# ojcharles/WeightedLD

Hardware: AMD Instinct MI355X
Metric: LD site-pairs/sec at N=2000 seq × L=20000 var sites; 1/2/4/8 GPU; %HBM roofline (higher is better)
Workload: dtype fp6 (e2m3) weights x fp4 (e2m1) codes on block-scaled MFMA, screen (f32 sums, exact on the rounded weights; rigorous f32 r2 bound over every pair); candidate tiles (0 of 49144): f32 sums in lib.rs's order on f32 MFMA, f32 epilogue

## Files before the change

include/weightedld.h:

```cpp
#ifndef WEIGHTEDLD_H
#define WEIGHTEDLD_H

#include <stddef.h>
#include <stdint.h>

#ifdef __cplusplus
extern "C" {
#endif

#define WLD_OK 0
#define WLD_E_ARG (-1)
#define WLD_E_HIP (-2)
#define WLD_E_OOM (-3)
#define WLD_E_NODEV (-4)
#define WLD_E_IO (-5)
#define WLD_E_FORMAT (-6)
#define WLD_E_STATE (-7)

#define WLD_SYM_A 0
#define WLD_SYM_C 1
#define WLD_SYM_G 2
#define WLD_SYM_T 3
#define WLD_SYM_MISSING 4
#define WLD_SYM_UNKNOWN 5
// ... 51 lines not shown
#define WLD_OPT_MFMA_LAYOUT 5
#define WLD_OPT_VALU_PLAIN 6
#define WLD_OPT_STAGING_ROWS 7
#define WLD_OPT_HOST_BATCH_PAIRS 8
#define WLD_OPT_REF_SUMS 11
#define WLD_OPT_FUSED_SCAN 12
#define WLD_OPT_SCREEN_FP6 13
#define WLD_OPT_TEST_GUARD 14
#define WLD_OPT_FP6_PAIRS_MIN_TILES 15
#define WLD_OPT_I8_PAIRS 16
#define WLD_OPT_FP6_A4 17
#define WLD_OPT_TARGET_BATCH_SLOTS 18
#define WLD_OPT_FP6_SHARED 19
#define WLD_OPT_PARTNERS_BATCH_BYTES 20
#define WLD_OPT_FP6_THREE 21
int wld_set_option(wld_ctx *ctx, int option, int64_t value);
int wld_get_option(wld_ctx *ctx, int option, int64_t *value);

int wld_set_window(wld_ctx *ctx, uint64_t max_distance, uint64_t max_sites);
int wld_get_window(wld_ctx *ctx, uint64_t *max_distance, uint64_t *max_sites);
int wld_window_pairs_in_chunks(wld_ctx *ctx, uint32_t begin, uint32_t end, uint64_t *pairs);
int wld_shard_chunks_window(wld_ctx *ctx, int n_shards, int shard, uint32_t *begin, uint32_t *end);
int wld_window_limits_copy(wld_ctx *ctx, uint32_t *hi);

typedef struct {
    uint64_t n;
    uint32_t *site_a;
    uint32_t *site_b;
    float *d;
    float *d_prime;
// ... 61 lines not shown
    int mfma_planes;
    uint64_t tiles;
    uint64_t candidate_tiles;
    double screen_ms;
    int screened;
    int ref_sums;
    uint64_t candidate_blocks;
    uint64_t candidate_pairs;
    int screen_fp6;
    int fp6_sampled;
    uint64_t progress_filled;
    int fp6_a4;
    int fp6_shared;
    int fp6_three;
    uint64_t fp6_rechecked;
} wld_run_stats;
int wld_last_stats(wld_ctx *ctx, wld_run_stats *out);
int wld_fp6_weight_codes(wld_ctx *ctx, uint8_t *codes, int *fits_fp4);

typedef struct {
    uint64_t n_sites;
    uint64_t bin_width;
    uint32_t n_bins;
    uint64_t pairs, none_pairs, nonfinite_pairs, counted_pairs;
    double r2_sum;
    double *score;
    uint32_t *partners;
    uint64_t *bin_pairs;
    double *bin_r2_sum;
    double kernel_ms;
// ... 133 lines not shown
```

weightedld_amd/_lib.py:

```python
import ctypes
import os

PKG_DIR = os.path.dirname(os.path.abspath(__file__))
LIB_PATH = os.environ.get("WLD_LIB_PATH") or os.path.join(PKG_DIR, "libweightedld.so")

WLD_OK = 0
STATUS = {
    -1: "WLD_E_ARG",
    -2: "WLD_E_HIP",
    -3: "WLD_E_OOM",
    -4: "WLD_E_NODEV",
    -5: "WLD_E_IO",
    -6: "WLD_E_FORMAT",
    -7: "WLD_E_STATE",
}
KERNEL_AUTO, KERNEL_VALU, KERNEL_MFMA = 0, 1, 2
OPTIONS = {"prefilter": 1, "screen": 2, "tile_order": 3, "all_planes": 4, "mfma_layout": 5, "valu_plain": 6,
           "staging_rows": 7, "host_batch_pairs": 8, "ref_sums": 11, "fused_scan": 12, "screen_fp6": 13,
           "test_guard": 14, "fp6_pairs_min_tiles": 15, "i8_pairs": 16, "fp6_a4": 17,
           "target_batch_slots": 18, "fp6_shared": 19, "partners_batch_bytes": 20, "fp6_three": 21}


class WldError(RuntimeError):
    def __init__(self, status, where, message):
        self.status = status
        self.name = STATUS.get(status, str(status))
        super().__init__("%s: %s (%s)" % (where, message, self.name))


class Pairs(ctypes.Structure):
    _fields_ = [
        ("n", ctypes.c_uint64),
        ("site_a", ctypes.POINTER(ctypes.c_uint32)),
        ("site_b", ctypes.POINTER(ctypes.c_uint32)),
        ("d", ctypes.POINTER(ctypes.c_float)),
# ... 15 lines not shown
        ("mfma_planes", ctypes.c_int),
        ("tiles", ctypes.c_uint64),
        ("candidate_tiles", ctypes.c_uint64),
        ("screen_ms", ctypes.c_double),
        ("screened", ctypes.c_int),
        ("ref_sums", ctypes.c_int),
        ("candidate_blocks", ctypes.c_uint64),
        ("candidate_pairs", ctypes.c_uint64),
        ("screen_fp6", ctypes.c_int),
        ("fp6_sampled", ctypes.c_int),
        ("progress_filled", ctypes.c_uint64),
        ("fp6_a4", ctypes.c_int),
        ("fp6_shared", ctypes.c_int),
        ("fp6_three", ctypes.c_int),
        ("fp6_rechecked", ctypes.c_uint64),
    ]


class Summary(ctypes.Structure):
    _fields_ = [
        ("n_sites", ctypes.c_uint64),
        ("bin_width", ctypes.c_uint64),
        ("n_bins", ctypes.c_uint32),
        ("pairs", ctypes.c_uint64),
        ("none_pairs", ctypes.c_uint64),
        ("nonfinite_pairs", ctypes.c_uint64),
        ("counted_pairs", ctypes.c_uint64),
        ("r2_sum", ctypes.c_double),
        ("score", ctypes.POINTER(ctypes.c_double)),
        ("partners", ctypes.POINTER(ctypes.c_uint32)),
# ... 283 lines not shown
```

weightedld_amd/csrc/capi.hip:

```cpp
#include <algorithm>
#include <cmath>
#include <chrono>
#include <condition_variable>
#include <cstdlib>
#include <cstring>
#include <deque>
#include <functional>
#include <mutex>
#include <string>
#include <thread>
#include <vector>

#include "common.hpp"
#include "tile_order.hpp"
#include "window_plan.hpp"
#include "summary_plan.hpp"
#include "heatmap_plan.hpp"
#include "annot_plan.hpp"
#include "blocks_plan.hpp"
#include "partners_plan.hpp"
#include "prune_plan.hpp"
#include "targets_plan.hpp"
#include "kernels.hpp"
#include "fp6_scale.hpp"
// ... 75 lines not shown
    unsigned long long *d_hcnt = nullptr;
    int cand_set = 0;
    int kernel_pref = WLD_KERNEL_AUTO;
    bool opt_prefilter = true, opt_tile_rows = false, opt_all_planes = false;
    int opt_screen = 1;
    screen_policy::Learned learned;
    screen_policy::Plan pass;
    DevBuf fp6_probe_buf;
    bool opt_site_major = false, opt_valu_plain = false;
    bool opt_fused_scan = true;
    int opt_test_guard = 0;
    int64_t opt_fp6_pairs_min = 0;
    bool opt_i8_pairs = true;
    int opt_fp6 = 1;
    bool opt_fp6_a4 = true;
    int opt_fp6_three = 1;
    bool opt_fp6_shared = true;
    bool opt_ref_sums = true;
    uint64_t opt_staging_rows = 1ull << 25, opt_host_batch_pairs = 1ull << 31;
    uint64_t opt_target_slots = targets_plan::kDefaultBatchSlots;
    uint64_t opt_partners_bytes = partners_plan::kDefaultBatchBytes;

    bool loaded = false;
    size_t L = 0, N = 0, LP = 0, NP = 0;
    DevBuf raw, wraw, codes, w_pad, wstats, site_ok, site_map, planes, frag;
    DevBuf rcodes, rw;
    DevBuf w6, f6a, f6b, f6marg;
    DevBuf w4;
    Fp6Screen f6{};
    DevBuf i8a, i8b;
// ... 517 lines not shown
double ref_extra_residual(const wld_ctx *c) {
    const double u = 0x1p-24, m = (double)(c->N / 8) + 16.0;
    const double gamma = m * u / (1.0 - m * u);
    double qsum = 0.0;
    for (int p = 0; p < 4; ++p) qsum += std::ldexp((double)c->wst.dsum[p], 8 * p);
    const double r = 9.0 * gamma * (qsum + 0.5 * (double)c->N) + 0.5 * (double)c->N;
    return r * (1.0 + 1e-9) + 1.0;
}

struct PolicyInputs {
    screen_policy::Options opt;
    screen_policy::LoadFacts load;
    screen_policy::PassFacts pass;
};
PolicyInputs policy_inputs(const wld_ctx *c, float thr, bool dense) {
    return {{c->opt_screen, c->opt_fp6, c->opt_ref_sums, c->opt_prefilter, c->opt_i8_pairs, c->opt_fp6_three},
            {c->kernel == WLD_KERNEL_MFMA, c->use_frag, c->wst.nonneg != 0, c->NP, c->plane_mask, c->fp6_ok,
             c->fp6_better},
            {c->f6_n_pairs != 0, c->n_tiles, thr, dense, c->prog_pass, c->pend.count_out != nullptr}};
}

ValuLaunch ref_valu_launch(wld_ctx *c, float thr) {
    return ValuLaunch{ptr<uint8_t>(c->rcodes), ptr<float>(c->rw), ptr<uint8_t>(c->site_ok), ptr<uint32_t>(c->tiles),
                      c->n_tiles, nullptr, (uint32_t)c->L, (uint32_t)c->NPr, chunk_rows_of(c->L), thr, c->safe, false,
                      true, c->ref_cls, (uint32_t)(c->N % 8)};
}

MfmaLaunch mfma_base(wld_ctx *c, float thr) {
    MfmaLaunch m{};
    m.wplanes = ptr<int8_t>(c->planes);
    m.tiles = ptr<uint32_t>(c->tiles);
// ... 33 lines not shown
        launch_pair_valu(ValuLaunch{ptr<uint8_t>(c->codes), ptr<float>(c->w_pad), ptr<uint8_t>(c->site_ok),
                                    ptr<uint32_t>(c->tiles), c->n_tiles, nullptr, (uint32_t)c->L, (uint32_t)c->NP,
                                    chunk_rows_of(c->L), thr, c->safe, c->opt_valu_plain, false, 0, 0},
                         o, dense, c->stream);
    } else {
        MfmaLaunch m = mfma_base(c, thr);
        m.codes = ptr<uint8_t>(c->codes);
        m.frag = c->use_frag ? ptr<uint8_t>(c->frag) : nullptr;
        m.frag_b = c->use_frag ? ptr<uint8_t>(c->frag) + c->LP * c->NP : nullptr;
        m.shift = c->shift;
        m.plane_mask = c->plane_mask;
        m.route = plan.route;
        m.bound_test = plan.bound_test;
        m.fp6_bail = plan.fp6_bail;
        m.fp6_three = plan.fp6_three;
        m.f6_rechecked = reinterpret_cast<unsigned *>(ptr<unsigned long long>(c->counters) + kF6Rechecked);
        m.i8img = &c->i8s;
        for (int t = 0; t < 3; ++t) m.resid[t] = c->wst.resid[t];
        for (int p = 0; p < 4; ++p) m.dsum[p] = c->wst.dsum[p];
        m.cand_list = ptr<uint32_t>(c->cand);
        unsigned long long *set = ptr<unsigned long long>(c->counters) + kCandSet0 + kCandSetWords * c->cand_set;
        m.cand_count = reinterpret_cast<unsigned *>(set);
        m.cand_work = reinterpret_cast<unsigned *>(ptr<unsigned long long>(c->counters) + 2) + 1;
        m.cand_buckets = reinterpret_cast<unsigned *>(set + 1);
        m.test_guard = c->opt_test_guard;
        if (scan && !dense) m.scan = *scan;
        RefRowsLaunch rr{};
        if (c->opt_ref_sums) {
            m.ref_valu = &rv;
            m.r_extra_q = ref_extra_residual(c);
// ... 148 lines not shown
            c->learned.reset();
            break;
        case WLD_OPT_FP6_A4:
            c->opt_fp6_a4 = value != 0;
            c->fp6_ok = c->fp6_better = c->fp6_tried = false;
            break;
        case WLD_OPT_FP6_SHARED:
            c->opt_fp6_shared = value != 0;
            c->fp6_ok = c->fp6_better = c->fp6_tried = false;
            break;
        case WLD_OPT_FP6_THREE:
            if (value < 0 || value > 2) return fail(WLD_E_ARG, "WLD_OPT_FP6_THREE takes 0 to 2");
            c->opt_fp6_three = (int)value;
            c->learned.reset();
            break;
        default: return fail(WLD_E_ARG, "unknown option %d", option);
    }
    return WLD_OK;
}

int wld_fp6_weight_codes(wld_ctx *c, uint8_t *codes, int *fits_fp4) {
    if (!c || !codes || !fits_fp4) return fail(WLD_E_ARG, "null argument");
    if (!c->members.empty()) return fail(WLD_E_ARG, "wld_fp6_weight_codes takes a single-device context");
    if (c->pend.active) return fail(WLD_E_STATE, "wld_fp6_weight_codes during a run");
    if (!c->loaded || !c->fp6_ok) return fail(WLD_E_STATE, "the loaded set has no fp6 operands");
    HIP_TRY(hipSetDevice(c->device));
    HIP_TRY(hipMemcpyAsync(codes, c->w6.p, c->N, hipMemcpyDeviceToHost, c->stream));
    HIP_TRY(hipStreamSynchronize(c->stream));
    *fits_fp4 = fp6_codes_fit_fp4(codes, c->N) ? 1 : 0;
    return WLD_OK;
// ... 83 lines not shown
        case WLD_OPT_MFMA_LAYOUT: *value = c->opt_site_major; break;
        case WLD_OPT_VALU_PLAIN: *value = c->opt_valu_plain; break;
        case WLD_OPT_REF_SUMS: *value = c->opt_ref_sums; break;
        case WLD_OPT_STAGING_ROWS: *value = (int64_t)c->opt_staging_rows; break;
        case WLD_OPT_HOST_BATCH_PAIRS: *value = (int64_t)c->opt_host_batch_pairs; break;
        case WLD_OPT_TARGET_BATCH_SLOTS: *value = (int64_t)c->opt_target_slots; break;
        case WLD_OPT_PARTNERS_BATCH_BYTES: *value = (int64_t)c->opt_partners_bytes; break;
        case WLD_OPT_FUSED_SCAN: *value = c->opt_fused_scan; break;
        case WLD_OPT_TEST_GUARD: *value = c->opt_test_guard; break;
        case WLD_OPT_FP6_PAIRS_MIN_TILES: *value = c->opt_fp6_pairs_min; break;
        case WLD_OPT_SCREEN_FP6: *value = c->opt_fp6; break;
        case WLD_OPT_I8_PAIRS: *value = c->opt_i8_pairs; break;
        case WLD_OPT_FP6_A4: *value = c->opt_fp6_a4; break;
        case WLD_OPT_FP6_SHARED: *value = c->opt_fp6_shared; break;
        case WLD_OPT_FP6_THREE: *value = c->opt_fp6_three; break;
        default: return fail(WLD_E_ARG, "unknown option %d", option);
    }
    return WLD_OK;
}

int wld_load(wld_ctx *c, const uint8_t *sites, size_t n_sites, size_t n_seqs, const uint64_t *site_map,
             const float *weights) {
    if (c && !c->members.empty()) {
        const size_t G = c->members.size();
        std::vector<int> st(G, WLD_OK);
        std::vector<std::string> msg(G);
        std::vector<std::thread> th;
        for (size_t k = 0; k < G; ++k)
            th.emplace_back([&, k] {
                st[k] = wld_load(c->members[k], sites, n_sites, n_seqs, site_map, weights);
// ... 248 lines not shown
        launch_gather(o, ptr<uint32_t>(c->chunk_base), r.lin_begin, lin_count, chunk_rows_of(c->L), (uint32_t)c->L, 0,
                      cn, c->out_a.bytes / 4, c->has_map && !c->prune_run ? ptr<uint32_t>(c->site_map) : nullptr,
                      ptr<uint32_t>(c->out_a), ptr<uint32_t>(c->out_b), ptr<float>(c->out_d), ptr<float>(c->out_dp),
                      ptr<float>(c->out_r2), c->stream);
        HIP_TRY(hipGetLastError());
        HIP_TRY(hipEventRecord(c->ev[5], c->stream));
        c->gather_cap = c->out_a.bytes / 4;
    }
    return WLD_OK;
}

int fp6_sample(wld_ctx *c, float thr, bool operands_fresh) {
    const PolicyInputs in = policy_inputs(c, thr, false);
    if (!screen_policy::wants_sample(in.opt, in.load, in.pass, c->learned)) return WLD_OK;
    const hipStream_t s = !operands_fresh && c->own_stream ? c->own_stream : c->stream;
    WLD_TRY(ensure(c->fp6_probe_buf, 3 * sizeof(unsigned)));
    MfmaLaunch m = mfma_base(c, thr);
    m.fp6_three = c->opt_fp6_three != 0 && m.f6_pairs != nullptr;
    const uint32_t entries = m.f6_pairs ? m.f6_n_pairs : m.n_tiles;
    const uint32_t stride = std::max<uint32_t>(1, std::min<uint32_t>(64, entries / 256));
    launch_fp6_probe(m, ptr<unsigned>(c->fp6_probe_buf), stride, s);
    HIP_TRY(hipGetLastError());
    unsigned h[3] = {0, 0, 0};
    HIP_TRY(hipMemcpyAsync(h, c->fp6_probe_buf.p, sizeof(h), hipMemcpyDeviceToHost, s));
    HIP_TRY(hipStreamSynchronize(s));
    c->fp6_sampled = true;
    screen_policy::learn(c->learned, screen_policy::Sample{thr, h[0], h[1], m.fp6_three, h[2]});
    return WLD_OK;
}

int run_enqueue(wld_ctx *c, float thr, uint32_t lin_begin, uint32_t lin_end, unsigned long long *count_out) {
    const uint32_t n = chunk_rows_of(c->L);
    c->have_rows = false;
    c->pend.active = false;
    const bool fp6_fresh = !c->fp6_tried && c->opt_fp6 != 0;
    if (fp6_fresh) WLD_TRY(fp6_prepare(c));
    WLD_TRY(build_tiles(c, lin_begin, lin_end, true));
    c->fp6_sampled = false;
    WLD_TRY(fp6_sample(c, thr, fp6_fresh));
    const uint64_t pairs = run_pairs(c, lin_begin, lin_end);
    const uint32_t T = (uint32_t)(c->LP / kTile);
    const uint32_t n_chunks = n * (n + 1) / 2;
// ... 145 lines not shown
    c->spec_gather = rows > 0;
    c->gather_cap = 0;
    c->stats.kernel = c->kernel;
    c->stats.pairs = r.pairs;
    c->stats.rows = rows;
    c->times_pending = true;
    c->times_order_end = order_end;
    c->stats.pair_kernel_launches = c->n_tiles ? screen_policy::stat_launches(route) : 0;
    c->stats.tiles = c->tiles_windowed ? c->n_tiles_listed : c->n_tiles;
    c->stats.screened = screen_policy::stat_screened(route);
    c->stats.screen_fp6 = screen_policy::stat_screen_fp6(route) ? 1 : abandoned ? 2 : 0;
    c->stats.fp6_sampled = c->fp6_sampled ? 1 : 0;
    c->stats.fp6_a4 = c->stats.screen_fp6 == 1 && c->f6.a4 ? 1 : 0;
    c->stats.fp6_shared = c->stats.screen_fp6 == 1 && c->f6.shared ? 1 : 0;
    c->stats.fp6_three = c->stats.screen_fp6 == 1 ? screen_policy::stat_fp6_three(c->pass) : 0;
    c->stats.fp6_rechecked = c->stats.fp6_three ? __atomic_load_n(&c->h_cnt[5], __ATOMIC_ACQUIRE) : 0;
    c->stats.candidate_pairs = cand_pairs ? h[0] : 0;
    screen_policy::learn(c->learned, screen_policy::Outcome{route, r.thr, false, h[2], c->n_tiles, h[0], r.pairs});
    c->stats.candidate_tiles = screened ? h[2] : c->n_tiles;
    c->stats.candidate_blocks = screened && !cand_pairs ? h[3] : 16 * (uint64_t)c->n_tiles;
    if (n_rows) *n_rows = rows;
    return WLD_OK;
}

int run_chunks(wld_ctx *c, float thr, uint32_t lin_begin, uint32_t lin_end, uint64_t *n_rows) {
    WLD_TRY(run_enqueue(c, thr, lin_begin, lin_end, nullptr));
    return run_complete(c, n_rows);
}
}

int wld_run(wld_ctx *c, float thr, uint32_t rb, uint32_t re, uint64_t *n_rows) {
// ... 1992 lines not shown
```

weightedld_amd/csrc/kernels.hpp:

```cpp
#pragma once

#include <hip/hip_runtime.h>

#include <cstdint>
#include <vector>

#include "screen_policy.hpp"

namespace wld {

constexpr int kChunk = 256;
constexpr int kTile = 64;
constexpr int kSeqPad = 64;
constexpr int kTilesPerChunk = kChunk / kTile;
constexpr uint32_t kNoTile = 0xFFFFFFFFu;

constexpr uint8_t kCodeIn = 1;
constexpr uint8_t kCodeMaj = 2;

struct OrderArgs {
    uint32_t *st_a, *st_b;
    float *st_d, *st_dp, *st_r2;
    uint64_t st_capacity;
    uint8_t *seg_cnt;
// ... 275 lines not shown
    uint32_t *cand_list;
    unsigned *cand_count;
    unsigned *cand_buckets;
    int test_guard = 0;
    unsigned *cand_work;
    const ValuLaunch *ref_valu;
    double r_extra_q;
    const RefRowsLaunch *ref_rows;
    ScanArgs scan;
    const Fp6Screen *fp6;
    uint32_t fp6_bail;
    const uint32_t *f6_pairs;
    uint32_t f6_n_pairs;
    bool fp6_three = false;
    unsigned *f6_rechecked = nullptr;
    const I8Screen *i8img = nullptr;
};
void launch_fp6_probe(const MfmaLaunch &m, unsigned *probe, uint32_t stride, hipStream_t s);
void launch_pair_mfma(const MfmaLaunch &m, const OrderArgs &o, const DenseArgs *dense, hipStream_t s,
                      hipEvent_t screen_done);

void launch_progress_init(unsigned *chunk_left, uint32_t lin_begin, uint32_t count, uint32_t n_chunk_rows, uint32_t L,
                          unsigned *prog_n, hipStream_t s);
void launch_progress_init_window(unsigned *chunk_left, uint32_t lin_begin, uint32_t count, uint32_t n_chunk_rows,
                                 const uint32_t *tiles, uint32_t n_tiles, unsigned *prog_n, hipStream_t s);
void launch_window_limits(const uint32_t *pos, uint32_t L, uint32_t LP, uint64_t D, uint64_t K, uint32_t *hi,
                          hipStream_t s);
void launch_run_init(unsigned long long *counters, uint32_t *chunk_total, uint32_t n_chunks, hipStream_t s);
void launch_chunk_scan(const ScanArgs &a, hipStream_t s);
void launch_gather(const OrderArgs &o, const uint32_t *chunk_base, uint32_t lin_begin, uint32_t count,
// ... 33 lines not shown
```

weightedld_amd/csrc/pair_common.hpp:

```cpp
#pragma once

#include "kernels.hpp"

namespace wld {

#ifndef WLD_EPI_DIVT
#define WLD_EPI_DIVT 1
#endif
__host__ __device__ __forceinline__ double recip_f64(double t, double r0) {
    double r = r0;
    double e = fma(-t, r, 1.0);
    r = fma(r, e, r);
    e = fma(-t, r, 1.0);
    return fma(r, e, r);
}
__host__ __forceinline__ double recip_seed_host(float t) {
    return fabsf(t) < 0x1p-126f ? (double)(1.0f / (t * 0x1p64f)) * 0x1p64 : (double)(1.0f / t);
}
__host__ __device__ __forceinline__ void ld_epilogue(float total_weight, float PA, float PB, float ld3, float &d_out,
                                                     float &dp_out, float &r2_out) {
    float ld_obs0, ld_obs1, ld_obs2, ld_obs3 = ld3;
    float Pa = total_weight - PA;
    float Pb = total_weight - PB;
    ld_obs2 = PA - ld_obs3;
// ... 146 lines not shown
    return F6tCol{col + mb, col - mb, fmaf(2.0f, mb, -R2), 2.0f * Mb, mb, col};
}
__host__ __device__ __forceinline__ float r2_screen_terms_f6t(float p, float s, float t, const F6tRow &a,
                                                              const F6tCol &b, float thr_c, float E, float &mlo) {
    const float d = s - t;
    const float m1 = a.c1 - d, m2 = (a.rA2 + b.cB2) + d;
    const float m3 = fmaf(2.0f, p, a.rA + b.cB3), m4 = fmaf(-2.0f, p, b.c4);
    mlo = fminf(fminf(m1, m2), fminf(m3, m4));
    const float cap2 = fminf(fmaf(-2.0f, p, a.Ma2), b.Mb2 - d);
    const float q = -((a.ma2 - s) * (b.mb - p));
    const float X0lo = p + (a.row + b.col);
    const float nt = fmaxf(fabsf(fmaf(X0lo, t, q)), fabsf(fmaf(X0lo + cap2, t, q)));
    const float nub = fmaf(2.0f, nt, E);
    return fmaf(nub, nub, -(thr_c * ((m1 * m2) * (m3 * m4))));
}
__host__ __device__ __forceinline__ float r2_screen_violation(float T, float A, float B, float AB, float R,
                                                              float thr_c) {
    float E, mloc, t2;
    screen_consts(T, R, E, mloc);
    const float t1 = r2_screen_terms(T, A, B, AB, R, thr_c, E, mloc, t2);
    return fmaxf(t1, t2);
}
__host__ __device__ __forceinline__ bool r2_screen_skip_f32(float T, float A, float B, float AB, float R, float thr) {
    return r2_screen_violation(T, A, B, AB, R, thr * (1.0f - 0x1p-7f)) <= 0.0f;
}
constexpr uint32_t kScreenF32MaxNP = 32768;

__device__ __forceinline__ void glds16(const void *gsrc, uint32_t lds_dst) {
    uint32_t keep;
    asm volatile(
// ... 101 lines not shown
        *a.cursor = 0;
        unsigned cand = 0, blocks = 0;
        if (a.cand_count) {
            cand = ld32(a.cand_count);
            blocks = ld32(a.cand_count + 1);
        }
        if (a.cursor_seen) *a.cursor_seen = (cand & kAbandonBit) ? ~0ull : cur;
        if (a.cand_reset) a.cand_reset[0] = a.cand_reset[1] = 0;
        if (a.cand_buckets_reset)
            for (int b = 0; b < 16; ++b) a.cand_buckets_reset[b] = 0;
        if (a.host_out) {
            a.host_out[0] = cur;
            a.host_out[1] = run;
            a.host_out[2] = cand;
            a.host_out[3] = blocks;
            if (a.rechecked) a.host_out[5] = ld32(a.rechecked);
            __threadfence_system();
        }
        if (a.rechecked) *a.rechecked = 0;
    }
    __syncthreads();
    unsigned long long base = sw[wv] + v - s;
    if (in_regs) {
#pragma unroll
        for (uint32_t j = 0; j < kScanRegs; ++j)
            if (lo + j < hi) {
                ct[lo + j] = 0;
                a.chunk_base[lo + j] = (uint32_t)base;
                base += vals[j];
            }
        return;
    }
    for (uint32_t i = lo; i < hi; ++i) {
        const uint32_t t = ld32(ct + i);
// ... 56 lines not shown
```

weightedld_amd/csrc/pair_mfma.hip:

```cpp
#include <algorithm>
#include <type_traits>
#include <vector>

#include "fp6_pack.hpp"
#include "pair_common.hpp"


namespace wld {

typedef int v4i __attribute__((ext_vector_type(4)));
typedef int v16i __attribute__((ext_vector_type(16)));

bool mfma_supported() { return true; }

namespace {
constexpr int kGroup = 8;
constexpr int kStageCodes = 4096;
constexpr int kDigStage = 128;
constexpr int kMaxPlanes = 4;
constexpr uint32_t kPlanes012 = 0 | (1 << 2) | (2 << 4);
constexpr int kDigGroup = 1024;
template <int NPL>
struct GroupShape {
    static constexpr int kStages = NPL == 1 ? 4 : kGroup;
// ... 844 lines not shown
    }
    bool doubt = false;
#pragma unroll
    for (int e = 0; e < 4; ++e) {
        const float2 a = sA[16 * ep.wq + 4 * (ep.lane >> 4) + e];
        const F6tRow ra = f6t_row(W6, a.x, a.y, ep.R2);
#pragma unroll
        for (int n = 0; n < 4; ++n) {
            float mlo;
            const float t1 = terms(ra, n, e, mlo);
            if (ep.valid_pair(4 * n + e) && (t1 > 0.0f || !(mlo >= ep.mloc))) doubt = true;
        }
    }
    return doubt;
}
}

template <int kFmt>
__global__ __launch_bounds__(256, 4) void pair_fp6_screen_kernel(const uint8_t *__restrict__ a6,
                                                                  const uint8_t *__restrict__ b6,
                                                                  const float2 *__restrict__ marg, float W6,
                                                                  const uint64_t *__restrict__ ok_bits,
                                                                  const uint32_t *__restrict__ tiles, uint32_t n_tiles,
                                                                  uint32_t NK, uint32_t L, uint32_t n_chunk_rows,
                                                                  float thr, OrderArgs o, ScreenArgs sc, float wv) {
    using F = F6Fmt<kFmt>;
    constexpr int kF6AStage = F::kAStage, kF6ABytes = F::kABytes, kF6Stage = F::kStage;
    __shared__ __attribute__((aligned(16))) uint8_t smem[2 * kF6Stage];
    __shared__ float2 sMarg[2 * kTile];
    __shared__ unsigned long long sMask;
// ... 74 lines not shown
        screen_verdict((uint32_t)sMask, ta, tb, tid, n_chunk_rows, o, sc);
    } else {
        screen_verdict(0u, ta, tb, tid, n_chunk_rows, o, sc);
    }
}

constexpr uint32_t kF6Single = 0x8000u;

#ifdef WLD_EXP_CLOCK
constexpr uint32_t kF6ClockSlots = 8192;
__device__ unsigned long long gF6Clock[2 * kF6ClockSlots];
extern "C" int wld_debug_f6_clock(unsigned long long *out) {
    return (int)hipMemcpyFromSymbol(out, HIP_SYMBOL(gF6Clock), sizeof(gF6Clock));
}
#endif
template <int kFmt, bool kThree = false>
__global__ __launch_bounds__(256, 3) void pair_fp6_screen2w_kernel(
    const uint8_t *__restrict__ a6, const uint8_t *__restrict__ b6, const float2 *__restrict__ marg, float W6,
    const uint64_t *__restrict__ ok_bits,
    const uint32_t *__restrict__ pairs, uint32_t n_pairs, uint32_t NK, uint32_t L, uint32_t n_chunk_rows, float thr,
    OrderArgs o, ScreenArgs sc, float wv) {
    using F = F6Fmt<kFmt>;
    constexpr int kF6AStage = F::kAStage, kF6ABytes = F::kABytes, kF6PStage = F::kPStage;
    __shared__ __attribute__((aligned(16))) uint8_t smem[2 * kF6PStage];
    __shared__ float2 sMarg[3 * kTile];
    __shared__ unsigned long long sMask[2];
    __shared__ uint32_t sBail, sCand[2];
    __shared__ uint32_t sDoubt[2];
    if (!sc.probe && blockIdx.x == 0 && threadIdx.x == 0) *sc.cand_work = 0u;
    const uint32_t tid = threadIdx.x, lane = tid & 63, wave = __builtin_amdgcn_readfirstlane(tid >> 6);
    const uint32_t half = wave >> 1, rp = wave & 1, ltid = tid & 127;
    const uint32_t lds = lds_addr(smem), lane16 = lane * 16;
    const uint32_t ei = sc.probe ? blockIdx.x * sc.probe_stride + blockIdx.x % sc.probe_stride : blockIdx.x;
    const uint32_t entry = ei < n_pairs ? pairs[ei] : kNoTile;
    if (entry == kNoTile) return;
    constexpr int kAPieces = kFmt == kF6A6 ? 3 : kFmt == kF6A4 ? 2 : 1;
    static_assert(kF6AStage == kAPieces * 4096 && kF6BStage == 4096, "five (fp4 A: four, shared: three) pieces per wave and stage");
    struct Src {
        const uint8_t *pA, *pB0, *pB1;
    };
    auto src_of = [&](uint32_t e) {
        const uint32_t ta_ = e >> 16, tb0_ = e & 0x7FFFu;
        Src r;
// ... 21 lines not shown
        const uint32_t tb = tb0 + (idle ? 0u : half);
        if (tid < 3 * kTile) {
            const uint32_t t = tid < kTile ? ta : tb0 + ((tid >= 2 * kTile && !single) ? 1u : 0u);
            sMarg[tid] = marg[t * kTile + (tid & (kTile - 1))];
        }
        if (tid == 0) {
            uint32_t v = 0;
            if (sc.bail) {
                const unsigned cc = __hip_atomic_load(sc.cand_count, __ATOMIC_RELAXED, __HIP_MEMORY_SCOPE_AGENT);
                v = cc > sc.bail ? ((cc & kAbandonBit) ? 2u : 1u) : 0u;
            }
            sBail = v;
        }
        if constexpr (kThree)
            if (tid < 2) sDoubt[tid] = 0u;
        asm volatile("s_waitcnt lgkmcnt(0)" ::: "memory");
        const uint64_t okA = ok_bits[ta], okB = ok_bits[tb];
        v4f acc[2][4][2][2];
        const uint32_t boff = kF6AStage + (idle ? 0u : half) * kF6BStage;
        const uint32_t aoff = 2 * rp * kF6ABytes;
        auto stage = [&](uint32_t kb, auto first) -> bool {
            constexpr bool kFirst = decltype(first)::value;
            asm volatile("s_waitcnt vmcnt(0)" ::: "memory");
            __builtin_amdgcn_s_barrier();
            asm volatile("" ::: "memory");
            if (kFirst) {
                if (sBail) {
                    if (tid == 0 && sBail == 1) {
                        atomicOr(sc.cand_count, kAbandonBit);
                        atomicOr(sc.cand_buckets, kAbandonBit);
// ... 35 lines not shown
#ifdef WLD_EXP_CLOCK
        const unsigned long long ck0 = clock64(), rt0 = wall_clock64();
#endif
        if (!stage(0, std::true_type{})) return;
        for (uint32_t kb = 1; kb < NK; ++kb) stage(kb, std::false_type{});
#ifdef WLD_EXP_CLOCK
        if (tid == 0) {
            gF6Clock[2 * (blockIdx.x % kF6ClockSlots)] = clock64() - ck0;
            gF6Clock[2 * (blockIdx.x % kF6ClockSlots) + 1] = wall_clock64() - rt0;
        }
#endif
        const F6Epi ep0{ta, tb, 2 * rp, lane, okA, okB, 2.0f * sc.Rf, thr * (1.0f - 0x1p-7f), sc.E, sc.mloc};
        const F6Epi ep1{ta, tb, 2 * rp + 1, lane, okA, okB, 2.0f * sc.Rf, thr * (1.0f - 0x1p-7f), sc.E, sc.mloc};
        if constexpr (kThree) {
            const float2 *sB = sMarg + kTile * (1 + half);
            const bool doubt = !idle && (f6t_any_doubt<F::kShared>(acc[0], ep0, sMarg, sB, W6, wv) ||
                                         f6t_any_doubt<F::kShared>(acc[1], ep1, sMarg, sB, W6, wv));
            if (doubt) sDoubt[half] = 1u;
            __syncthreads();
#ifdef WLD_EXP_ZERO_IMG
            const bool again = (sDoubt[0] | sDoubt[1]) == 0x5EEDu;
#else
            const bool again = (sDoubt[0] | sDoubt[1]) != 0;
#endif
            if (!again) {
                if (sc.probe) {
                    if (ltid == 0 && !idle) atomicAdd(sc.probe + 1, 1u);
                } else if (!idle) {
                    screen_verdict(0u, ta, tb, ltid, n_chunk_rows, o, sc);
                }
                return;
            }
            if (unsigned *const cnt = sc.probe ? sc.probe + 2 : sc.rechecked; tid == 0 && cnt) atomicAdd(cnt, 1u);
#pragma unroll
// ... 337 lines not shown
    const uint32_t grid = std::min<uint32_t>(m.n_tiles, kCandidateGrid);
    launch_lds_planes<kModePrefilter, true>(n, m, ok_bits, m.cand_list, 0, m.cand_count, grid, idx, o, dn, sc, s);
}
}

namespace {
void fp6_screen_args(const MfmaLaunch &m, ScreenArgs &sc) {
    sc.R = std::ceil(m.fp6->R * 32.0) / 32.0;
    sc.Rf = (float)sc.R;
    sc.f32 = 2;
    screen_consts(m.fp6->Tg, 2.0f * sc.Rf, sc.E, sc.mloc);
}
template <int kFmt>
void launch_fp6_screen_fmt(const MfmaLaunch &m, const uint64_t *ok_bits, const OrderArgs &o, const ScreenArgs &sc,
                           uint32_t stride, hipStream_t s) {
    if (m.f6_pairs && m.fp6_three) {
        hipLaunchKernelGGL((pair_fp6_screen2w_kernel<kFmt, true>), dim3((m.f6_n_pairs + stride - 1) / stride),
                           dim3(256), 0, s, m.fp6->a6, m.fp6->b6, reinterpret_cast<const float2 *>(m.fp6->marg),
                           m.fp6->W6, ok_bits, m.f6_pairs, m.f6_n_pairs, m.fp6->NK, m.L, m.n_chunk_rows, m.thr, o, sc,
                           m.fp6->wv);
    } else if (m.f6_pairs) {
        hipLaunchKernelGGL(pair_fp6_screen2w_kernel<kFmt>, dim3((m.f6_n_pairs + stride - 1) / stride), dim3(256), 0, s,
                           m.fp6->a6, m.fp6->b6, reinterpret_cast<const float2 *>(m.fp6->marg), m.fp6->W6, ok_bits,
                           m.f6_pairs, m.f6_n_pairs, m.fp6->NK, m.L, m.n_chunk_rows,
                           m.thr, o, sc, m.fp6->wv);
    } else {
        hipLaunchKernelGGL(pair_fp6_screen_kernel<kFmt>, dim3((m.n_tiles + stride - 1) / stride), dim3(256), 0, s,
                           m.fp6->a6, m.fp6->b6, reinterpret_cast<const float2 *>(m.fp6->marg), m.fp6->W6, ok_bits,
                           m.tiles, m.n_tiles, m.fp6->NK, m.L, m.n_chunk_rows, m.thr,
                           o, sc, m.fp6->wv);
    }
// ... 4 lines not shown
        launch_fp6_screen_fmt<kF6Shared>(m, ok_bits, o, sc, stride, s);
    else if (m.fp6->a4)
        launch_fp6_screen_fmt<kF6A4>(m, ok_bits, o, sc, stride, s);
    else
        launch_fp6_screen_fmt<kF6A6>(m, ok_bits, o, sc, stride, s);
}
}

void launch_fp6_probe(const MfmaLaunch &m, unsigned *probe, uint32_t stride, hipStream_t s) {
    const uint64_t *ok_bits = reinterpret_cast<const uint64_t *>(m.wplanes + okbits_offset(m.NP));
    ScreenArgs sc{};
    sc.nonneg = m.nonneg;
    fp6_screen_args(m, sc);
    sc.probe = probe;
    sc.probe_stride = std::max<uint32_t>(stride, 1);
    (void)hipMemsetAsync(probe, 0, 3 * sizeof(unsigned), s);
    launch_fp6_screen(m, ok_bits, OrderArgs{}, sc, sc.probe_stride, s);
}

void launch_pair_mfma(const MfmaLaunch &m, const OrderArgs &o, const DenseArgs *dense, hipStream_t s,
                      hipEvent_t screen_done) {
    using screen_policy::Route;
    const DenseArgs dn = dense ? *dense : DenseArgs{nullptr, nullptr, nullptr, nullptr};
    const uint64_t *ok_bits = reinterpret_cast<const uint64_t *>(m.wplanes + okbits_offset(m.NP));
    ScreenArgs sc{0.0,         0.0f,         0.0f,      0.0f,        0, m.nonneg, m.cand_list, m.cand_count,
                  m.cand_list + 16 * (size_t)m.n_tiles, m.cand_work, m.cand_buckets, m.n_tiles, 0, ScanArgs{}};
    if (!m.frag) {
        const dim3 g(m.n_tiles), b(256);
        if (dense)
            hipLaunchKernelGGL((pair_mfma_rows_kernel<kModeDense>), g, b, 0, s, m.codes, m.wplanes, ok_bits, m.tiles,
                               m.L, m.NP, m.n_chunk_rows, m.thr, m.shift, o, dn, sc);
// ... 101 lines not shown
```

weightedld_amd/csrc/screen_policy.hpp:

```cpp
#pragma once
#include <algorithm>
#include <cmath>
#include <cstdint>

namespace wld {
namespace screen_policy {

enum class Route : uint8_t {
    F32Plain,
    F32RefOrder,
    IntAll,
    Fp6Screen,
    I8PairScreen,
    I8TileScreen,
    TwoPlaneScreen,
    CandidatePairs,
};


constexpr uint64_t kFp6Keep = 16;
constexpr uint64_t kOnePlaneKeep = 2;
constexpr uint64_t kTwoPlaneKeep = 5;
constexpr uint64_t kCandidatePairsKeep = 10;
constexpr uint32_t kSampleMinTiles = 2048;
constexpr uint64_t kFp6ThreeKeep = 8;

struct Learned {
    float screen_bad = -1.0f;
    float screen2_bad = -1.0f;
    float ref_pairs_bad = -1.0f;
    float fp6_bad = -1.0f;
    float fp6_good = INFINITY;
    float fp6_three_good = INFINITY;

    void reset() { *this = Learned{}; }
};

struct Options {
    int screen;
    int fp6;
    bool ref_sums, prefilter, i8_pairs;
    int fp6_three = 1;
};
struct LoadFacts {
    bool mfma;
    bool use_frag;
    bool nonneg;
    uint64_t NP;
    unsigned plane_mask;
    bool fp6_ok, fp6_better;
};
struct PassFacts {
    bool have_pairs;
    uint32_t n_tiles;
    float thr;
    bool dense;
    bool prog_pass;
    bool count_out;
};

struct Plan {
    Route route = Route::F32Plain;
    bool bound_test = false;
    uint32_t fp6_bail = 0;
    bool i8_images = false;
    bool fp6_three = false;
};

static inline bool fp6_three(const Options &o, const PassFacts &p, const Learned &s) {
    if (!p.have_pairs) return false;
    return o.fp6_three == 2 || (o.fp6_three == 1 && p.thr >= s.fp6_three_good);
}

static inline Plan decide(const Options &o, const LoadFacts &l, const PassFacts &p, const Learned &s) {
    Plan plan;
    const float thr = p.thr;
    const bool bound = o.prefilter && thr > 0.0f;
    const bool ref_screen = o.ref_sums && l.mfma && !p.dense && l.use_frag && bound && o.screen != 0;
    if (o.ref_sums && !ref_screen) {
        plan.route = Route::F32RefOrder;
        return plan;
    }
    if (!l.mfma) return plan;
    plan.route = Route::IntAll;
    plan.bound_test = bound;
    if (!bound || p.dense || !l.use_frag) return plan;

    const bool one = o.screen == 2 || o.screen == 3 || (o.screen == 1 && thr > s.screen_bad);
    const bool two = __builtin_popcount(l.plane_mask & 15) >= 3 &&
                     (o.screen == 3 || (o.screen == 1 && !one && !ref_screen && thr > s.screen2_bad));
    if (two) {
        plan.route = Route::TwoPlaneScreen;
    } else if (one) {
        const bool fp6_auto = o.fp6 == 1 || o.fp6 == 3;
        if (l.fp6_ok && (o.fp6 == 2 || (fp6_auto && l.fp6_better && thr > s.fp6_bad))) {
            plan.route = Route::Fp6Screen;
            plan.fp6_three = fp6_three(o, p, s);
            if (fp6_auto && !p.prog_pass && !p.count_out)
                plan.fp6_bail = std::max<uint32_t>(p.n_tiles / (uint32_t)kFp6Keep, 1);
        } else if (o.i8_pairs && p.have_pairs && l.nonneg && l.NP <= 16384) {
            plan.route = Route::I8PairScreen;
            plan.i8_images = true;
        } else {
            plan.route = Route::I8TileScreen;
        }
    } else if (ref_screen) {
        if (!((o.screen == 1 && thr > s.ref_pairs_bad) || o.screen == 4)) return Plan{Route::F32RefOrder};
        plan.route = Route::CandidatePairs;
    }
    return plan;
}

// ... 8 lines not shown
    return planned;
}

static inline bool wants_sample(Options o, const LoadFacts &l, PassFacts p, const Learned &s) {
    if (o.screen == 3) o.screen = 2;
    p.dense = false;
    return o.fp6 == 1 && decide(o, l, p, s).route == Route::Fp6Screen && p.n_tiles >= kSampleMinTiles &&
           !(p.thr >= s.fp6_good);
}

struct Sample {
    float thr;
    uint64_t candidates, sampled;
    bool three = false;
    uint64_t rechecked = 0;
};
static inline void learn(Learned &s, const Sample &r) {
    if (r.candidates * kFp6Keep > r.sampled) {
        s.fp6_bad = std::max(s.fp6_bad, r.thr);
        return;
    }
    s.fp6_good = std::min(s.fp6_good, r.thr);
    if (r.three && r.sampled && r.rechecked * kFp6ThreeKeep <= (r.sampled + 1) / 2)
        s.fp6_three_good = std::min(s.fp6_three_good, r.thr);
}

struct Outcome {
    Route route;
    float thr;
    bool abandoned;
    uint64_t candidate_tiles;
    uint64_t n_tiles;
    uint64_t candidate_pairs;
    uint64_t pairs;
};
static inline void learn(Learned &s, const Outcome &r) {
    if (r.abandoned) {
        s.fp6_bad = std::max(s.fp6_bad, r.thr);
        return;
// ... 7 lines not shown
        s.screen2_bad = std::max(s.screen2_bad, r.thr);
    if (r.route == Route::CandidatePairs && r.candidate_pairs * kCandidatePairsKeep > r.pairs)
        s.ref_pairs_bad = std::max(s.ref_pairs_bad, r.thr);
}


static inline bool ran_screen(Route r) {
    return r == Route::Fp6Screen || r == Route::I8PairScreen || r == Route::I8TileScreen ||
           r == Route::TwoPlaneScreen || r == Route::CandidatePairs;
}
static inline int stat_screened(Route r) {
    return r == Route::CandidatePairs ? 4 : r == Route::TwoPlaneScreen ? 3 : ran_screen(r) ? 1 : 0;
}
static inline int stat_screen_fp6(Route r) { return r == Route::Fp6Screen ? 1 : 0; }
static inline int stat_fp6_three(const Plan &p) { return p.route == Route::Fp6Screen && p.fp6_three ? 1 : 0; }
static inline int stat_launches(Route r) { return r == Route::CandidatePairs ? 3 : ran_screen(r) ? 2 : 1; }

}
}
```

Measured before the change: 485.0 billion.

## Add quick per-wave fp6 screen bound ahead of the per-pair three-sum test

Adds a coarse per-wave bound that takes maxima of the accumulated sums and minima of the row and column margins. When the bound proves no pair in a row block can pass, the per-pair three-sum doubt test is skipped for that block. A sampling probe counts how often the full test is still needed, and the learned policy turns the quick path on by default only when that fraction is low enough. This adds extra VALU work and an atomic counter in the epilogue, and it helps only when most blocks can be rejected by the coarse bound.

```diff
diff --git a/include/weightedld.h b/include/weightedld.h
--- a/include/weightedld.h
+++ b/include/weightedld.h
@@ -89,6 +89,7 @@
 #define WLD_OPT_FP6_SHARED 19
 #define WLD_OPT_PARTNERS_BATCH_BYTES 20
 #define WLD_OPT_FP6_THREE 21
+#define WLD_OPT_FP6_QUICK 22
 int wld_set_option(wld_ctx *ctx, int option, int64_t value);
 int wld_get_option(wld_ctx *ctx, int option, int64_t *value);
 
@@ -180,6 +181,8 @@
     int fp6_shared;
     int fp6_three;
     uint64_t fp6_rechecked;
+    int fp6_quick;
+    uint64_t fp6_quick_full;
 } wld_run_stats;
 int wld_last_stats(wld_ctx *ctx, wld_run_stats *out);
 int wld_fp6_weight_codes(wld_ctx *ctx, uint8_t *codes, int *fits_fp4);
diff --git a/weightedld_amd/_lib.py b/weightedld_amd/_lib.py
--- a/weightedld_amd/_lib.py
+++ b/weightedld_amd/_lib.py
@@ -18,7 +18,8 @@
 OPTIONS = {"prefilter": 1, "screen": 2, "tile_order": 3, "all_planes": 4, "mfma_layout": 5, "valu_plain": 6,
            "staging_rows": 7, "host_batch_pairs": 8, "ref_sums": 11, "fused_scan": 12, "screen_fp6": 13,
            "test_guard": 14, "fp6_pairs_min_tiles": 15, "i8_pairs": 16, "fp6_a4": 17,
-           "target_batch_slots": 18, "fp6_shared": 19, "partners_batch_bytes": 20, "fp6_three": 21}
+           "target_batch_slots": 18, "fp6_shared": 19, "partners_batch_bytes": 20, "fp6_three": 21,
+           "fp6_quick": 22}
 
 
 class WldError(RuntimeError):
@@ -64,6 +65,8 @@
         ("fp6_shared", ctypes.c_int),
         ("fp6_three", ctypes.c_int),
         ("fp6_rechecked", ctypes.c_uint64),
+        ("fp6_quick", ctypes.c_int),
+        ("fp6_quick_full", ctypes.c_uint64),
     ]
 
 
diff --git a/weightedld_amd/csrc/capi.hip b/weightedld_amd/csrc/capi.hip
--- a/weightedld_amd/csrc/capi.hip
+++ b/weightedld_amd/csrc/capi.hip
@@ -113,6 +113,7 @@
     bool opt_i8_pairs = true;
     int opt_fp6 = 1;
     bool opt_fp6_a4 = true;
+    int opt_fp6_quick = 1;
     int opt_fp6_three = 1;
     bool opt_fp6_shared = true;
     bool opt_ref_sums = true;
@@ -660,7 +661,8 @@
     screen_policy::PassFacts pass;
 };
 PolicyInputs policy_inputs(const wld_ctx *c, float thr, bool dense) {
-    return {{c->opt_screen, c->opt_fp6, c->opt_ref_sums, c->opt_prefilter, c->opt_i8_pairs, c->opt_fp6_three},
+    return {{c->opt_screen, c->opt_fp6, c->opt_ref_sums, c->opt_prefilter, c->opt_i8_pairs, c->opt_fp6_three,
+             c->opt_fp6_quick},
             {c->kernel == WLD_KERNEL_MFMA, c->use_frag, c->wst.nonneg != 0, c->NP, c->plane_mask, c->fp6_ok,
              c->fp6_better},
             {c->f6_n_pairs != 0, c->n_tiles, thr, dense, c->prog_pass, c->pend.count_out != nullptr}};
@@ -724,6 +726,7 @@
         m.bound_test = plan.bound_test;
         m.fp6_bail = plan.fp6_bail;
         m.fp6_three = plan.fp6_three;
+        m.fp6_quick = plan.fp6_quick;
         m.f6_rechecked = reinterpret_cast<unsigned *>(ptr<unsigned long long>(c->counters) + kF6Rechecked);
         m.i8img = &c->i8s;
         for (int t = 0; t < 3; ++t) m.resid[t] = c->wst.resid[t];
@@ -902,6 +905,11 @@
             c->opt_fp6_three = (int)value;
             c->learned.reset();
             break;
+        case WLD_OPT_FP6_QUICK:
+            if (value < 0 || value > 2) return fail(WLD_E_ARG, "WLD_OPT_FP6_QUICK takes 0 to 2");
+            c->opt_fp6_quick = (int)value;
+            c->learned.reset();
+            break;
         default: return fail(WLD_E_ARG, "unknown option %d", option);
     }
     return WLD_OK;
@@ -1015,6 +1023,7 @@
         case WLD_OPT_FP6_A4: *value = c->opt_fp6_a4; break;
         case WLD_OPT_FP6_SHARED: *value = c->opt_fp6_shared; break;
         case WLD_OPT_FP6_THREE: *value = c->opt_fp6_three; break;
+        case WLD_OPT_FP6_QUICK: *value = c->opt_fp6_quick; break;
         default: return fail(WLD_E_ARG, "unknown option %d", option);
     }
     return WLD_OK;
@@ -1293,18 +1302,19 @@
     const PolicyInputs in = policy_inputs(c, thr, false);
     if (!screen_policy::wants_sample(in.opt, in.load, in.pass, c->learned)) return WLD_OK;
     const hipStream_t s = !operands_fresh && c->own_stream ? c->own_stream : c->stream;
-    WLD_TRY(ensure(c->fp6_probe_buf, 3 * sizeof(unsigned)));
+    WLD_TRY(ensure(c->fp6_probe_buf, 4 * sizeof(unsigned)));
     MfmaLaunch m = mfma_base(c, thr);
     m.fp6_three = c->opt_fp6_three != 0 && m.f6_pairs != nullptr;
+    m.fp6_quick = m.fp6_three && c->opt_fp6_quick != 0;
     const uint32_t entries = m.f6_pairs ? m.f6_n_pairs : m.n_tiles;
     const uint32_t stride = std::max<uint32_t>(1, std::min<uint32_t>(64, entries / 256));
     launch_fp6_probe(m, ptr<unsigned>(c->fp6_probe_buf), stride, s);
     HIP_TRY(hipGetLastError());
-    unsigned h[3] = {0, 0, 0};
+    unsigned h[4] = {0, 0, 0, 0};
     HIP_TRY(hipMemcpyAsync(h, c->fp6_probe_buf.p, sizeof(h), hipMemcpyDeviceToHost, s));
     HIP_TRY(hipStreamSynchronize(s));
     c->fp6_sampled = true;
-    screen_policy::learn(c->learned, screen_policy::Sample{thr, h[0], h[1], m.fp6_three, h[2]});
+    screen_policy::learn(c->learned, screen_policy::Sample{thr, h[0], h[1], m.fp6_three, h[2], m.fp6_quick, h[3]});
     return WLD_OK;
 }
 
@@ -1480,7 +1490,10 @@
     c->stats.fp6_a4 = c->stats.screen_fp6 == 1 && c->f6.a4 ? 1 : 0;
     c->stats.fp6_shared = c->stats.screen_fp6 == 1 && c->f6.shared ? 1 : 0;
     c->stats.fp6_three = c->stats.screen_fp6 == 1 ? screen_policy::stat_fp6_three(c->pass) : 0;
-    c->stats.fp6_rechecked = c->stats.fp6_three ? __atomic_load_n(&c->h_cnt[5], __ATOMIC_ACQUIRE) : 0;
+    const unsigned long long f6_counts = __atomic_load_n(&c->h_cnt[5], __ATOMIC_ACQUIRE);
+    c->stats.fp6_rechecked = c->stats.fp6_three ? (f6_counts & 0xFFFFFFFFull) : 0;
+    c->stats.fp6_quick = c->stats.screen_fp6 == 1 ? screen_policy::stat_fp6_quick(c->pass) : 0;
+    c->stats.fp6_quick_full = c->stats.fp6_quick ? (f6_counts >> 32) : 0;
     c->stats.candidate_pairs = cand_pairs ? h[0] : 0;
     screen_policy::learn(c->learned, screen_policy::Outcome{route, r.thr, false, h[2], c->n_tiles, h[0], r.pairs});
     c->stats.candidate_tiles = screened ? h[2] : c->n_tiles;
diff --git a/weightedld_amd/csrc/kernels.hpp b/weightedld_amd/csrc/kernels.hpp
--- a/weightedld_amd/csrc/kernels.hpp
+++ b/weightedld_amd/csrc/kernels.hpp
@@ -313,6 +313,7 @@
     uint32_t f6_n_pairs;
     bool fp6_three = false;
     unsigned *f6_rechecked = nullptr;
+    bool fp6_quick = false;
     const I8Screen *i8img = nullptr;
 };
 void launch_fp6_probe(const MfmaLaunch &m, unsigned *probe, uint32_t stride, hipStream_t s);
diff --git a/weightedld_amd/csrc/pair_common.hpp b/weightedld_amd/csrc/pair_common.hpp
--- a/weightedld_amd/csrc/pair_common.hpp
+++ b/weightedld_amd/csrc/pair_common.hpp
@@ -184,6 +184,46 @@
     const float nub = fmaf(2.0f, nt, E);
     return fmaf(nub, nub, -(thr_c * ((m1 * m2) * (m3 * m4))));
 }
+struct F6qAcc {
+    float dmax = 0.0f, pmax = 0.0f, nt = 0.0f;
+};
+struct F6qRowMin {
+    float c1, rA2, rA;
+};
+struct F6qColMin {
+    float cB2, cB3, c4;
+};
+__host__ __device__ __forceinline__ void f6q_row_min(F6qRowMin &m, const F6tRow &a) {
+    m.c1 = fminf(m.c1, a.c1);
+    m.rA2 = fminf(m.rA2, a.rA2);
+    m.rA = fminf(m.rA, a.rA);
+}
+__host__ __device__ __forceinline__ F6qColMin f6q_col_min(const F6tCol (&b)[4]) {
+    return F6qColMin{fminf(fminf(b[0].cB2, b[1].cB2), fminf(b[2].cB2, b[3].cB2)),
+                     fminf(fminf(b[0].cB3, b[1].cB3), fminf(b[2].cB3, b[3].cB3)),
+                     fminf(fminf(b[0].c4, b[1].c4), fminf(b[2].c4, b[3].c4))};
+}
+__host__ __device__ __forceinline__ float f6q_pair(float p, float s, float t, const F6tRow &a, const F6tCol &b,
+                                                   F6qAcc &acc) {
+    const float d = s - t;
+    acc.dmax = fmaxf(acc.dmax, d);
+    acc.pmax = fmaxf(acc.pmax, p);
+    const float q = -((a.ma2 - s) * (b.mb - p));
+    const float X0lo = p + (a.row + b.col);
+    const float cap2 = fminf(fmaf(-2.0f, p, a.Ma2), b.Mb2 - d);
+    const float nt = fmaxf(fabsf(fmaf(X0lo, t, q)), fabsf(fmaf(X0lo + cap2, t, q)));
+    acc.nt = fmaxf(acc.nt, nt);
+    return nt;
+}
+__host__ __device__ __forceinline__ float f6q_lane_terms(const F6qAcc &acc, const F6qRowMin &a, const F6qColMin &b,
+                                                         float thr_c, float E, float &mlo) {
+    const float m1 = a.c1 - acc.dmax, m2 = a.rA2 + b.cB2;
+    const float m3 = a.rA + b.cB3, m4 = fmaf(-2.0f, acc.pmax, b.c4);
+    mlo = fminf(fminf(m1, m2), fminf(m3, m4));
+    const float nub = fmaf(2.0f, acc.nt, E);
+    return fmaf(nub, nub, -(thr_c * ((m1 * m2) * (m3 * m4))));
+}
+__host__ __device__ __forceinline__ bool f6q_skip(float t1, float mlo, float mloc) { return t1 <= 0.0f && mlo >= mloc; }
 __host__ __device__ __forceinline__ float r2_screen_violation(float T, float A, float B, float AB, float R,
                                                               float thr_c) {
     float E, mloc, t2;
@@ -315,10 +355,11 @@
             a.host_out[1] = run;
             a.host_out[2] = cand;
             a.host_out[3] = blocks;
-            if (a.rechecked) a.host_out[5] = ld32(a.rechecked);
+            if (a.rechecked)
+                a.host_out[5] = (unsigned long long)ld32(a.rechecked) | (unsigned long long)ld32(a.rechecked + 1) << 32;
             __threadfence_system();
         }
-        if (a.rechecked) *a.rechecked = 0;
+        if (a.rechecked) a.rechecked[0] = a.rechecked[1] = 0;
     }
     __syncthreads();
     unsigned long long base = sw[wv] + v - s;
diff --git a/weightedld_amd/csrc/pair_mfma.hip b/weightedld_amd/csrc/pair_mfma.hip
--- a/weightedld_amd/csrc/pair_mfma.hip
+++ b/weightedld_amd/csrc/pair_mfma.hip
@@ -882,6 +882,59 @@
     }
     return doubt;
 }
+template <bool kShared>
+__device__ __forceinline__ bool f6t_quick_skip(const v4f (&acc)[4][2][2], const F6Epi &ep, const float2 *sA,
+                                               const F6tCol (&cb)[4], const F6qColMin &cm, float W6, float wv) {
+    F6qRowMin rm{INFINITY, INFINITY, INFINITY};
+    F6qAcc q;
+#pragma unroll
+    for (int e = 0; e < 4; ++e) {
+        const float2 a = sA[16 * ep.wq + 4 * (ep.lane >> 4) + e];
+        const F6tRow ra = f6t_row(W6, a.x, a.y, ep.R2);
+        f6q_row_min(rm, ra);
+#pragma unroll
+        for (int n = 0; n < 4; ++n) {
+            float p = acc[n][0][1][e], s = acc[n][1][0][e], t = acc[n][1][1][e];
+            if constexpr (kShared) p *= 0.5f * wv, s *= wv, t *= wv;
+            f6q_pair(p, s, t, ra, cb[n], q);
+            __builtin_amdgcn_sched_barrier(0);
+        }
+    }
+    float mlo;
+    const float t1 = f6q_lane_terms(q, rm, cm, ep.thr_c, ep.E, mlo);
+    return __ballot(!f6q_skip(t1, mlo, ep.mloc)) == 0;
+}
+template <bool kShared, bool kQuick>
+__device__ __forceinline__ bool f6t_wave_doubt(v4f (&acc)[2][4][2][2], const F6Epi &ep0, const F6Epi &ep1,
+                                               const float2 *sA, const float2 *sB, float W6, float wv, uint32_t *full) {
+    if constexpr (kQuick) {
+        bool full0 = true, full1 = true;
+        if (ep0.ta != ep0.tb) {
+            F6tCol cb[4];
+#pragma unroll
+            for (int n = 0; n < 4; ++n) {
+                const float2 b = sB[(ep0.lane & 15) + 16 * n];
+                cb[n] = f6t_col(b.x, b.y, ep0.R2);
+            }
+            const F6qColMin cm = f6q_col_min(cb);
+            full0 = !f6t_quick_skip<kShared>(acc[0], ep0, sA, cb, cm, W6, wv);
+            full1 = !f6t_quick_skip<kShared>(acc[1], ep1, sA, cb, cm, W6, wv);
+            if ((full0 || full1) && ep0.lane == 0) atomicAdd(full, (uint32_t)full0 + (uint32_t)full1);
+        }
+        uint32_t lane = ep0.lane;
+        asm volatile("" : "+v"(lane), "+s"(wv)::"memory");
+#pragma unroll
+        for (int j = 0; j < 2; ++j)
+#pragma unroll
+            for (int n = 0; n < 4; ++n) asm volatile("" : "+v"(acc[j][n][1][1]));
+        F6Epi e0 = ep0, e1 = ep1;
+        e0.lane = e1.lane = lane;
+        return (full0 && f6t_any_doubt<kShared>(acc[0], e0, sA, sB, W6, wv)) ||
+               (full1 && f6t_any_doubt<kShared>(acc[1], e1, sA, sB, W6, wv));
+    }
+    return f6t_any_doubt<kShared>(acc[0], ep0, sA, sB, W6, wv) ||
+           f6t_any_doubt<kShared>(acc[1], ep1, sA, sB, W6, wv);
+}
 }
 
 template <int kFmt>
@@ -986,7 +1039,7 @@
     return (int)hipMemcpyFromSymbol(out, HIP_SYMBOL(gF6Clock), sizeof(gF6Clock));
 }
 #endif
-template <int kFmt, bool kThree = false>
+template <int kFmt, bool kThree = false, bool kQuick = false>
 __global__ __launch_bounds__(256, 3) void pair_fp6_screen2w_kernel(
     const uint8_t *__restrict__ a6, const uint8_t *__restrict__ b6, const float2 *__restrict__ marg, float W6,
     const uint64_t *__restrict__ ok_bits,
@@ -999,6 +1052,8 @@
     __shared__ unsigned long long sMask[2];
     __shared__ uint32_t sBail, sCand[2];
     __shared__ uint32_t sDoubt[2];
+    __shared__ uint32_t sQuickFull;
+    static_assert(kThree || !kQuick, "the quick test stands in front of the three-sum test");
     if (!sc.probe && blockIdx.x == 0 && threadIdx.x == 0) *sc.cand_work = 0u;
     const uint32_t tid = threadIdx.x, lane = tid & 63, wave = __builtin_amdgcn_readfirstlane(tid >> 6);
     const uint32_t half = wave >> 1, rp = wave & 1, ltid = tid & 127;
@@ -1050,6 +1105,8 @@
         }
         if constexpr (kThree)
             if (tid < 2) sDoubt[tid] = 0u;
+        if constexpr (kQuick)
+            if (tid == 2) sQuickFull = 0u;
         asm volatile("s_waitcnt lgkmcnt(0)" ::: "memory");
         const uint64_t okA = ok_bits[ta], okB = ok_bits[tb];
         v4f acc[2][4][2][2];
@@ -1115,10 +1172,14 @@
         const F6Epi ep1{ta, tb, 2 * rp + 1, lane, okA, okB, 2.0f * sc.Rf, thr * (1.0f - 0x1p-7f), sc.E, sc.mloc};
         if constexpr (kThree) {
             const float2 *sB = sMarg + kTile * (1 + half);
-            const bool doubt = !idle && (f6t_any_doubt<F::kShared>(acc[0], ep0, sMarg, sB, W6, wv) ||
-                                         f6t_any_doubt<F::kShared>(acc[1], ep1, sMarg, sB, W6, wv));
+            const bool doubt =
+                !idle && f6t_wave_doubt<F::kShared, kQuick>(acc, ep0, ep1, sMarg, sB, W6, wv, &sQuickFull);
             if (doubt) sDoubt[half] = 1u;
             __syncthreads();
+            if constexpr (kQuick) {
+                unsigned *const cnt = sc.probe ? sc.probe + 3 : sc.rechecked ? sc.rechecked + 1 : nullptr;
+                if (tid == 0 && cnt && sQuickFull) atomicAdd(cnt, sQuickFull);
+            }
 #ifdef WLD_EXP_ZERO_IMG
             const bool again = (sDoubt[0] | sDoubt[1]) == 0x5EEDu;
 #else
@@ -1486,7 +1547,12 @@
 template <int kFmt>
 void launch_fp6_screen_fmt(const MfmaLaunch &m, const uint64_t *ok_bits, const OrderArgs &o, const ScreenArgs &sc,
                            uint32_t stride, hipStream_t s) {
-    if (m.f6_pairs && m.fp6_three) {
+    if (m.f6_pairs && m.fp6_three && m.fp6_quick) {
+        hipLaunchKernelGGL((pair_fp6_screen2w_kernel<kFmt, true, true>), dim3((m.f6_n_pairs + stride - 1) / stride),
+                           dim3(256), 0, s, m.fp6->a6, m.fp6->b6, reinterpret_cast<const float2 *>(m.fp6->marg),
+                           m.fp6->W6, ok_bits, m.f6_pairs, m.f6_n_pairs, m.fp6->NK, m.L, m.n_chunk_rows, m.thr, o, sc,
+                           m.fp6->wv);
+    } else if (m.f6_pairs && m.fp6_three) {
         hipLaunchKernelGGL((pair_fp6_screen2w_kernel<kFmt, true>), dim3((m.f6_n_pairs + stride - 1) / stride),
                            dim3(256), 0, s, m.fp6->a6, m.fp6->b6, reinterpret_cast<const float2 *>(m.fp6->marg),
                            m.fp6->W6, ok_bits, m.f6_pairs, m.f6_n_pairs, m.fp6->NK, m.L, m.n_chunk_rows, m.thr, o, sc,
@@ -1521,7 +1587,7 @@
     fp6_screen_args(m, sc);
     sc.probe = probe;
     sc.probe_stride = std::max<uint32_t>(stride, 1);
-    (void)hipMemsetAsync(probe, 0, 3 * sizeof(unsigned), s);
+    (void)hipMemsetAsync(probe, 0, 4 * sizeof(unsigned), s);
     launch_fp6_screen(m, ok_bits, OrderArgs{}, sc, sc.probe_stride, s);
 }
 
diff --git a/weightedld_amd/csrc/screen_policy.hpp b/weightedld_amd/csrc/screen_policy.hpp
--- a/weightedld_amd/csrc/screen_policy.hpp
+++ b/weightedld_amd/csrc/screen_policy.hpp
@@ -24,6 +24,8 @@
 constexpr uint64_t kCandidatePairsKeep = 10;
 constexpr uint32_t kSampleMinTiles = 2048;
 constexpr uint64_t kFp6ThreeKeep = 8;
+constexpr uint64_t kFp6QuickKeep = 4;
+constexpr uint64_t kFp6RowBlocksPerTile = 4;
 
 struct Learned {
     float screen_bad = -1.0f;
@@ -32,6 +34,7 @@
     float fp6_bad = -1.0f;
     float fp6_good = INFINITY;
     float fp6_three_good = INFINITY;
+    float fp6_quick_good = INFINITY;
 
     void reset() { *this = Learned{}; }
 };
@@ -41,6 +44,7 @@
     int fp6;
     bool ref_sums, prefilter, i8_pairs;
     int fp6_three = 1;
+    int fp6_quick = 1;
 };
 struct LoadFacts {
     bool mfma;
@@ -65,11 +69,16 @@
     uint32_t fp6_bail = 0;
     bool i8_images = false;
     bool fp6_three = false;
+    bool fp6_quick = false;
 };
 
 static inline bool fp6_three(const Options &o, const PassFacts &p, const Learned &s) {
     if (!p.have_pairs) return false;
     return o.fp6_three == 2 || (o.fp6_three == 1 && p.thr >= s.fp6_three_good);
+}
+
+static inline bool fp6_quick(const Options &o, const PassFacts &p, const Learned &s) {
+    return o.fp6_quick == 2 || (o.fp6_quick == 1 && p.thr >= s.fp6_quick_good);
 }
 
 static inline Plan decide(const Options &o, const LoadFacts &l, const PassFacts &p, const Learned &s) {
@@ -96,6 +105,7 @@
         if (l.fp6_ok && (o.fp6 == 2 || (fp6_auto && l.fp6_better && thr > s.fp6_bad))) {
             plan.route = Route::Fp6Screen;
             plan.fp6_three = fp6_three(o, p, s);
+            plan.fp6_quick = plan.fp6_three && fp6_quick(o, p, s);
             if (fp6_auto && !p.prog_pass && !p.count_out)
                 plan.fp6_bail = std::max<uint32_t>(p.n_tiles / (uint32_t)kFp6Keep, 1);
         } else if (o.i8_pairs && p.have_pairs && l.nonneg && l.NP <= 16384) {
@@ -134,6 +144,8 @@
     uint64_t candidates, sampled;
     bool three = false;
     uint64_t rechecked = 0;
+    bool quick = false;
+    uint64_t quick_full = 0;
 };
 static inline void learn(Learned &s, const Sample &r) {
     if (r.candidates * kFp6Keep > r.sampled) {
@@ -143,6 +155,8 @@
     s.fp6_good = std::min(s.fp6_good, r.thr);
     if (r.three && r.sampled && r.rechecked * kFp6ThreeKeep <= (r.sampled + 1) / 2)
         s.fp6_three_good = std::min(s.fp6_three_good, r.thr);
+    if (r.three && r.quick && r.sampled && r.quick_full * kFp6QuickKeep <= r.sampled * kFp6RowBlocksPerTile)
+        s.fp6_quick_good = std::min(s.fp6_quick_good, r.thr);
 }
 
 struct Outcome {
@@ -180,6 +194,7 @@
 }
 static inline int stat_screen_fp6(Route r) { return r == Route::Fp6Screen ? 1 : 0; }
 static inline int stat_fp6_three(const Plan &p) { return p.route == Route::Fp6Screen && p.fp6_three ? 1 : 0; }
+static inline int stat_fp6_quick(const Plan &p) { return stat_fp6_three(p) && p.fp6_quick ? 1 : 0; }
 static inline int stat_launches(Route r) { return r == Route::CandidatePairs ? 3 : ran_screen(r) ? 2 : 1; }
 
 }
```

New measurement: 510.3 billion (median of 6 runs). 1.05x the previous value.
